# tyiannak/pyAudioAnalysis

Hardware: NVIDIA H100
Metric: audio frames/sec short-term feature_extraction @16kHz 50/25ms (higher is better)
Workload: dtype f32

## Files before the change

### pyaudioanalysis_b200/csrc/b200aa.cu

```cuda
#include <cuda_runtime.h>
#include <nvtx3/nvToolsExt.h>

#include <algorithm>
#include <atomic>
#include <cmath>
#include <cstdio>
#include <cstring>
#include <map>
#include <memory>
#include <mutex>
#include <string>
#include <vector>

#include "../../include/b200aa.h"
#include "common.cuh"
#include "generic_kernel.cuh"
#include "fast_kernel.cuh"
#include "pair_kernel.cuh"
#include "solo_kernel.cuh"
#include "tables.inl"

using namespace b200aa;

static thread_local std::string g_cuda_err;
// ... 236 lines not shown
                if (cntg[g] < 3 && (best < 0 || load[g] < load[best])) best = g;
            grp[best * 3 + cntg[best]++] = f;
            load[best] += m_count[f];
        }
        bl.mel_grp = put_i(grp);
    }
    while (blob.size() % 4) blob.push_back(0);
    bl.words = (int)blob.size();
    return (rc_mel != B200AA_OK) ? rc_mel : rc_chr;
}

extern "C" int b200aa_plan_create(b200aa_plan **out, int fs, int window, int step)
{
    if (!out || fs <= 0 || window < 2 || step < 1) return B200AA_ERR_INVALID;
    int rc = b200aa_device_ok();
    if (rc != B200AA_OK) return rc;
    std::unique_ptr<b200aa_plan> pl(new b200aa_plan);
    pl->fs = fs; pl->window = window; pl->step = step; pl->K = window / 2;
    CK(cudaGetDevice(&pl->device));
    CK(cudaDeviceGetAttribute(&pl->sm_count, cudaDevAttrMultiProcessorCount, pl->device));
    pl->tables_status = build_blob(fs, pl->K, pl->h_blob, pl->bl);
    CK(cudaMalloc(&pl->d_blob, sizeof(int) * pl->h_blob.size()));
    CK(cudaMemcpy(pl->d_blob, pl->h_blob.data(), sizeof(int) * pl->h_blob.size(), cudaMemcpyHostToDevice));
    Transform *t = nullptr;
    rc = get_transform(pl.get(), window, &t);
    if (rc != B200AA_OK) return rc;
    rc = fast_plan_init(fs, window, step, pl->h_blob, pl->bl, &pl->fast, &pl->fast_kind);
    if (rc != B200AA_OK) return rc;
    int sl_ = 0, sr_ = 0;
    if ((pair_r_for_window(window) || solo_shape_for_window(window, &sl_, &sr_)) && pl->tables_status == B200AA_OK) {
        std::vector<double> mel, chr, dct;
        b200aa_host::build_mel(fs, pl->K, mel);
        b200aa_host::build_chroma(fs, pl->K, chr);
        b200aa_host::build_dct(dct);
        std::vector<int> pblob;
        PairBlobLayout pbl{};
        build_pair_blob(mel, chr, dct, pl->K, pblob, pbl);
        rc = pair_plan_init(window, pblob, pbl, &pl->pair);
        if (rc != B200AA_OK) return cuda_fail(cudaGetLastError(), "pair_plan_init");
        rc = solo_plan_init(window, pblob, pbl, &pl->solo);
        if (rc != B200AA_OK) return cuda_fail(cudaGetLastError(), "solo_plan_init");
    }
    CK(cudaMalloc(&pl->d_counters, b200aa_plan::kSlots * b200aa_plan::kSlotBytes));
    *out = pl.release();
    return B200AA_OK;
}

extern "C" void b200aa_plan_destroy(b200aa_plan *plan) { delete plan; }
static int slot_acquire(b200aa_plan *pl, cudaStream_t st, unsigned *slot, unsigned int **ctr)
{
    std::lock_guard<std::mutex> g(pl->slot_mu);
    const unsigned s = pl->next_slot++ % b200aa_plan::kSlots;
    if (!pl->slot_event[s]) CK(cudaEventCreateWithFlags(&pl->slot_event[s], cudaEventDisableTiming));
    if (pl->slot_used[s]) CK(cudaStreamWaitEvent(st, pl->slot_event[s], 0));
    *slot = s;
    *ctr = reinterpret_cast<unsigned int *>(pl->d_counters + size_t(s) * b200aa_plan::kSlotBytes);
    return B200AA_OK;
}
static int slot_done(b200aa_plan *pl, cudaStream_t st, unsigned slot)
{
    std::lock_guard<std::mutex> g(pl->slot_mu);
    CK(cudaEventRecord(pl->slot_event[slot], st));
    pl->slot_used[slot] = true;
    return B200AA_OK;
}

static bool use_pair(const b200aa_plan *pl) { return pl->pair.R && !pl->force_generic && (pl->prefer < 0 || pl->prefer == 2); }
static bool use_solo(const b200aa_plan *pl) { return pl->solo.L && !pl->force_generic && (pl->prefer < 0 || pl->prefer == 3); }
static bool use_fast(const b200aa_plan *pl) { return pl->fast_kind && !pl->force_generic && (pl->prefer < 0 || pl->prefer == 1); }
extern "C" int b200aa_plan_kernel_kind(const b200aa_plan *plan)
{
    if (!plan) return 0;
    return use_pair(plan) ? 2 : (use_solo(plan) ? 3 : (use_fast(plan) ? 1 : 0));
}
extern "C" int b200aa_plan_prefer_kernel(b200aa_plan *plan, int kind)
{
    if (!plan || kind < -1 || kind > 3) return B200AA_ERR_INVALID;
    plan->prefer = kind;
    return B200AA_OK;
}
static float *g_pair_dump = nullptr;
extern "C" int b200aa_debug_set_dump(float *d_rows)
{
    g_pair_dump = d_rows;
    return B200AA_OK;
}
extern "C" int b200aa_plan_force_generic(b200aa_plan *plan, int on)
{
    if (!plan) return 0;
    int prev = plan->force_generic;
    plan->force_generic = on ? 1 : 0;
    return prev;
}

extern "C" int b200aa_plan_trim(b200aa_plan *plan)
{
    if (!plan) return B200AA_ERR_INVALID;
    std::lock_guard<std::mutex> g(plan->host_mu);
    for (int i = 0; i < 4; ++i) {
        if (plan->ws[i]) cudaFree(plan->ws[i]);
        plan->ws[i] = nullptr; plan->ws_cap[i] = 0;
    }
    for (int k = 0; k < b200aa_plan::kPipe; ++k)
        for (int j = 0; j < 3; ++j) {
            if (plan->pipe_ws[k][j]) cudaFree(plan->pipe_ws[k][j]);
            plan->pipe_ws[k][j] = nullptr; plan->pipe_cap[k][j] = 0;
        }
    return B200AA_OK;
}

static int plan_device_check(const b200aa_plan *pl)
{
    int dev = -1;
    CK(cudaGetDevice(&dev));
    return dev == pl->device ? B200AA_OK : B200AA_ERR_INVALID;
}

__device__ __forceinline__ int float_key(float f)
{
    int b = __float_as_int(f);
    return b >= 0 ? b : b ^ 0x7fffffff;
}
__device__ __forceinline__ float key_float(int k) { return __int_as_float(k >= 0 ? k : k ^ 0x7fffffff); }

__global__ void stats_init_kernel(b200aa_clip_norm *nm, int64_t n)
{
    int64_t i = blockIdx.x * int64_t(blockDim.x) + threadIdx.x;
    if (i >= n) return;
    unsigned long long *acc = reinterpret_cast<unsigned long long *>(&nm[i].rsv[1]);
    *acc = 0ull;
    reinterpret_cast<int *>(&nm[i].lo)[0] = 0x7fffffff;
    reinterpret_cast<int *>(&nm[i].hi)[0] = int(0x80000000u);
}

template <int DTYPE>
__global__ void __launch_bounds__(256) stats_accum_kernel(const void *sig, int64_t n_samples, int64_t clip_stride,
                                                           const int64_t *len, b200aa_clip_norm *nm, int chunks)
{
    const int64_t b = blockIdx.y;
    const int64_t L = len ? len[b] : n_samples;
    const int64_t per = (L + chunks - 1) / chunks;
    const int64_t s0 = blockIdx.x * per, s1 = min(L, s0 + per);
    long long isum = 0;
    double dsum = 0.0;
    int kmin = 0x7fffffff, kmax = int(0x80000000u);
    if (DTYPE == B200AA_DTYPE_I16) {
        const short *x = reinterpret_cast<const short *>(sig) + b * clip_stride;
        int mn = 32767, mx = -32768;
        int64_t i = s0 + threadIdx.x;
        const bool al = ((reinterpret_cast<uintptr_t>(x + s0) & 15) == 0);
        if (al) {
            const int4 *v = reinterpret_cast<const int4 *>(x + s0);
            const int64_t nv = (s1 - s0) / 8;
            int64_t j = threadIdx.x;
            for (; j + 3 * int64_t(blockDim.x) < nv; j += 4 * int64_t(blockDim.x)) {
                int4 q[4];
#pragma unroll
                for (int t = 0; t < 4; ++t) q[t] = __ldg(v + j + t * int64_t(blockDim.x));
                int acc = 0;
#pragma unroll
                for (int t = 0; t < 4; ++t) {
                    const int w4[4] = {q[t].x, q[t].y, q[t].z, q[t].w};
#pragma unroll
                    for (int u = 0; u < 4; ++u) {
                        const int a0 = (short)(w4[u] & 0xffff), a1 = w4[u] >> 16;
                        acc += a0 + a1;
                        mn = min(mn, min(a0, a1));
                        mx = max(mx, max(a0, a1));
// ... 699 lines not shown
```

### pyaudioanalysis_b200/csrc/pair_kernel.cuh

```cuda
#pragma once
#include "common.cuh"
#include "dft_codelets.cuh"
#include <algorithm>
#include <cstring>
#include <utility>
#include "fast_kernel.cuh"
#include "sched.cuh"

namespace b200aa {

#ifndef B200AA_PAIR_MAXWARPS
#define B200AA_PAIR_MAXWARPS 24
#endif
constexpr int kPairMaxWarps = B200AA_PAIR_MAXWARPS;
#ifndef B200AA_PAIR_MINBLOCKS
#define B200AA_PAIR_MINBLOCKS 1
#endif
constexpr int kPairMinBlocks = B200AA_PAIR_MINBLOCKS;
#ifndef B200AA_SOLO_MAXWARPS
#define B200AA_SOLO_MAXWARPS 24
#endif
#ifndef B200AA_SOLO_MINBLOCKS
#define B200AA_SOLO_MINBLOCKS 1
#endif
// ... 201 lines not shown
        below += run > thr ? 0.f : 1.f;
#endif
    }
    const float sp = sp2.x + sp2.y, fl = fl2.x + fl2.y;
    __syncwarp();
    float e = 0.f;
    constexpr int MAXP = 2 * (Lb / CB + 2);
#pragma unroll
    for (int q = 0; q < MAXP; ++q) e += (dlv.y + q < dlv.z) ? parts[dlv.y + q] : 0.f;
    float ent = 0.f;
    if (l < 10) {
        const float sj = fdiv(e, sxx + B200AA_EPS);
        ent = -sj * flog2(sj + B200AA_EPS);
    }
    float q4;
    {
        const bool up8 = l & 8, up4 = l & 4;
        float k0_ = up8 ? below : sp, k1_ = up8 ? ent : fl;
        const float g0_ = up8 ? sp : below, g1_ = up8 ? fl : ent;
        k0_ += __shfl_xor_sync(0xffffffffu, g0_, 8);
        k1_ += __shfl_xor_sync(0xffffffffu, g1_, 8);
        float kk = up4 ? k1_ : k0_;
        const float gg = up4 ? k0_ : k1_;
        kk += __shfl_xor_sync(0xffffffffu, gg, 4);
        kk += __shfl_xor_sync(0xffffffffu, kk, 2);
        kk += __shfl_xor_sync(0xffffffffu, kk, 1);
        q4 = kk;
    }
    if (l == 0) {
        fv[3] = cen;
        fv[4] = sx > 0.f ? fsqrt_pos(fdiv(q4, sx)) : 0.f;
        fv[34] = sx;
        fv[35] = sxx;
    }
    if (l == 4) fv[6] = q4;
    if (l == 8) fv[7] = q4 >= float(K) ? 0.f : q4 * invK;
    if (l == 12) fv[5] = q4;
    __syncwarp();
}

template <int P, int NV, int D, int NA>
__device__ __forceinline__ void mr_halve(float (&v)[NA], int lane)
{
    if constexpr (P > 1) {
        constexpr int H = P / 2;
        const bool up = lane & D;
#pragma unroll
        for (int i = 0; i < H; ++i) {
            if (i < NV) {
                if (i + H < NV) {
                    const float keep = up ? v[i + H] : v[i], send = up ? v[i] : v[i + H];
                    v[i] = keep + __shfl_xor_sync(0xffffffffu, send, D);
                } else {
                    v[i] += __shfl_xor_sync(0xffffffffu, v[i], D);
                }
            }
        }
        mr_halve<H, (NV < H ? NV : H), D / 2, NA>(v, lane);
    } else {
#pragma unroll
        for (int d = D; d >= 1; d >>= 1) v[0] += __shfl_xor_sync(0xffffffffu, v[0], d);
    }
}
template <int NV>
struct MultiReduce {
    static constexpr int P0 = NV > 16 ? 32 : (NV > 8 ? 16 : 8);
    static constexpr int SH = NV > 16 ? 0 : (NV > 8 ? 1 : 2);
    __device__ static __forceinline__ void run(float (&v)[NV], int lane) { mr_halve<P0, NV, 16, NV>(v, lane); }
};

template <int R, bool FULL>
struct TdShape {
    using S = PairShape<R>;
    static constexpr int NREST = (S::N % 10) ? 1 : 0;
    static constexpr int NE = FULL ? 10 + NREST : 5;
    static constexpr int EB = FULL ? 0 : 5;
    static constexpr int NFIRST = FULL ? 0 : S::N / 2;
    static constexpr int ROW0 = NFIRST / 32, LANE0 = NFIRST % 32;
    static constexpr int ZROW0 = (!FULL && LANE0 == 0) ? ROW0 - 1 : ROW0;
    static_assert(FULL || S::kShareable, "half-frame sharing needs whole blocks per half");
};

template <int R, bool FULL, bool TWO>
__device__ __forceinline__ void td_frame(const float (&u)[R], float cm, const b200aa_clip_norm &nm, int lane,
                                         float *e , int &flips, int &link)
{
    using S = PairShape<R>;
    using Td = TdShape<R, FULL>;
    constexpr int N = S::N, Lt = S::Lt;
    unsigned prevP = 0u, prevQ = 0u;
    int fl = 0, lk = 0;
#pragma unroll
    for (int r = Td::ZROW0; r < R; ++r) {
        const float d = u[r] - cm;
        const unsigned P = __ballot_sync(0xffffffffu, d > nm.lo);
        unsigned Q = 0u;
        if (TWO) Q = __ballot_sync(0xffffffffu, d < nm.hi);
        if (FULL && r == 0) { prevP = (P & 1u) << 31; prevQ = (Q & 1u) << 31; }
        if (r >= Td::ROW0) {
            const int n0 = 32 * r;
            const int nstart = FULL ? 1 : Td::NFIRST;
            const unsigned valid = n0 >= nstart ? 0xffffffffu : (n0 + 32 <= nstart ? 0u : (0xffffffffu << (nstart - n0)));
            const unsigned cP = (P ^ __funnelshift_l(prevP, P, 1)) & valid;
            fl += __popc(cP);
            if (!FULL && r == Td::ROW0) lk += int((cP >> Td::LANE0) & 1u);
            if (TWO) {
                const unsigned cQ = (Q ^ __funnelshift_l(prevQ, Q, 1)) & valid;
                fl += __popc(cQ);
                if (!FULL && r == Td::ROW0) lk += int((cQ >> Td::LANE0) & 1u);
            }
            const float y = fmaf(nm.a, d, nm.bp);
            const bool live = !(r == Td::ROW0 && Td::LANE0 > 0) || lane >= Td::LANE0;
            const int b0 = (n0 / Lt) < 10 ? (n0 / Lt) : 10;
            const int end = b0 < 10 ? (b0 + 1) * Lt : N;
            const int thr = end - n0;
            const int i0 = b0 - Td::EB, i1 = (b0 + 1 < 10 ? b0 + 1 : 10) - Td::EB;
            if (thr >= 32) {
                if (i0 >= 0 && i0 < Td::NE) { if (live) e[i0] = fmaf(y, y, e[i0]); }
            } else {
                const bool first = lane < thr;
                if (i0 >= 0 && i0 < Td::NE) { if (live && first) e[i0] = fmaf(y, y, e[i0]); }
                if (i1 >= 0 && i1 < Td::NE) { if (live && !first) e[i1] = fmaf(y, y, e[i1]); }
            }
        }
        prevP = P; prevQ = Q;
    }
    flips = TWO ? fl : 2 * fl;
    link = TWO ? lk : 2 * lk;
}

template <int R, bool FULL, bool TWO>
__device__ __forceinline__ void td_pair(const float2 (&u)[R], float cm, const b200aa_clip_norm &nm, int lane,
                                        float2 *e2 , int &flips_a, int &link_a, int &flips_b, int &link_b)
{
    using S = PairShape<R>;
    using Td = TdShape<R, FULL>;
    constexpr int N = S::N, Lt = S::Lt;
    unsigned pPa = 0u, pQa = 0u, pPb = 0u, pQb = 0u;
    int fa = 0, la = 0, fb = 0, lb = 0;
    const float2 ncm = make_float2(-cm, -cm), a2 = make_float2(nm.a, nm.a), bp2 = make_float2(nm.bp, nm.bp);
#pragma unroll
    for (int r = Td::ZROW0; r < R; ++r) {
        const float2 d = f2add(u[r], ncm);
        const unsigned Pa = __ballot_sync(0xffffffffu, d.x > nm.lo), Pb = __ballot_sync(0xffffffffu, d.y > nm.lo);
        unsigned Qa = 0u, Qb = 0u;
        if (TWO) { Qa = __ballot_sync(0xffffffffu, d.x < nm.hi); Qb = __ballot_sync(0xffffffffu, d.y < nm.hi); }
        if (FULL && r == 0) { pPa = (Pa & 1u) << 31; pQa = (Qa & 1u) << 31; pPb = (Pb & 1u) << 31; pQb = (Qb & 1u) << 31; }
        if (r >= Td::ROW0) {
            const int n0 = 32 * r;
            const int nstart = FULL ? 1 : Td::NFIRST;
            const unsigned valid = n0 >= nstart ? 0xffffffffu : (n0 + 32 <= nstart ? 0u : (0xffffffffu << (nstart - n0)));
            const unsigned cPa = (Pa ^ __funnelshift_l(pPa, Pa, 1)) & valid, cPb = (Pb ^ __funnelshift_l(pPb, Pb, 1)) & valid;
            fa += __popc(cPa); fb += __popc(cPb);
            if (!FULL && r == Td::ROW0) { la += int((cPa >> Td::LANE0) & 1u); lb += int((cPb >> Td::LANE0) & 1u); }
            if (TWO) {
                const unsigned cQa = (Qa ^ __funnelshift_l(pQa, Qa, 1)) & valid, cQb = (Qb ^ __funnelshift_l(pQb, Qb, 1)) & valid;
                fa += __popc(cQa); fb += __popc(cQb);
                if (!FULL && r == Td::ROW0) { la += int((cQa >> Td::LANE0) & 1u); lb += int((cQb >> Td::LANE0) & 1u); }
            }
            const float2 y = f2fma(a2, d, bp2);
            const bool live = !(r == Td::ROW0 && Td::LANE0 > 0) || lane >= Td::LANE0;
            const int b0 = (n0 / Lt) < 10 ? (n0 / Lt) : 10;
            const int end = b0 < 10 ? (b0 + 1) * Lt : N;
            const int thr = end - n0;
            const int i0 = b0 - Td::EB, i1 = (b0 + 1 < 10 ? b0 + 1 : 10) - Td::EB;
            if (thr >= 32) {
                if (i0 >= 0 && i0 < Td::NE) { if (live) e2[i0] = f2fma(y, y, e2[i0]); }
            } else {
                const bool first = lane < thr;
                if (i0 >= 0 && i0 < Td::NE) { if (live && first) e2[i0] = f2fma(y, y, e2[i0]); }
                if (i1 >= 0 && i1 < Td::NE) { if (live && !first) e2[i1] = f2fma(y, y, e2[i1]); }
            }
        }
        pPa = Pa; pQa = Qa; pPb = Pb; pQb = Qb;
    }
    flips_a = TWO ? fa : 2 * fa; link_a = TWO ? la : 2 * la;
    flips_b = TWO ? fb : 2 * fb; link_b = TWO ? lb : 2 * lb;
}

__device__ __forceinline__ void frame_scale(float E, float inv_a2n, float &s, float &inv_s)
{
    const float t = E * inv_a2n;
    const int ex = (__float_as_int(t) >> 23) & 0xff;
    int k = (127 - ex) >> 1;
    k = k < -30 ? -30 : (k > 40 ? 40 : k);
    s = __int_as_float((127 + k) << 23);
    inv_s = __int_as_float((127 - k) << 23);
}

struct FeatTables {
    const float *dct;
    const int *mrec;
    const float4 *mw;
    const int2 *chr;
    int LQ, CT;
};

template <int K>
__device__ __forceinline__ void rows_to_features(const float *Xa, const float *Xb, const float *Xprev, bool fresh, float carried,
                                                 const int *dlane, float *parts, float *msraw, float *mslog, float *mfold, float *chr,
                                                 float *fva, float *fvb, const FeatTables &ft, int lane)
{
    const int half = lane >> 4, l16 = lane & 15;
    const unsigned FULLM = 0xffffffffu;
    {
        const float *X = half ? Xb : Xa;
        const float *Xp = half ? Xa : Xprev;
        pair_spectral<K>(X, Xp, carried, fresh, dlane + l16 * 4, parts + half * 32, half ? fvb : fva, l16, half);
    }
    {
        const float *X = half ? Xb : Xa;
        float acc = 0.f;
#pragma unroll 4
        for (int q = 0; q < ft.LQ; ++q) {
            const int rec = ft.mrec[q * 16 + l16];
            const float4 w = ft.mw[q * 16 + l16];
            const float *xp = X + (rec & 0xffff);
            acc = fmaf(xp[0], w.x, acc);
            acc = fmaf(xp[1], w.y, acc);
            acc = fmaf(xp[2], w.z, acc);
            acc = fmaf(xp[3], w.w, acc);
            if (rec & (1 << 24)) { msraw[half * B200AA_N_MEL + ((rec >> 16) & 0xff)] = acc; acc = 0.f; }
        }
        float ch = 0.f;
        for (int t = 0; t < ft.CT; ++t) {
            const int2 e = ft.chr[t * 16 + l16];
            const float v = X[e.x];
            ch = fmaf(v * v, __int_as_float(e.y), ch);
        }
        if (l16 < 12) chr[half * 12 + l16] = ch;
    }
    __syncwarp();
#pragma unroll
    for (int t = lane; t < 2 * B200AA_N_MEL; t += 32) mslog[t] = 0.30102999566398120f * flog2(msraw[t] + B200AA_EPS);
    __syncwarp();
#pragma unroll
    for (int t = lane; t < 2 * B200AA_N_MEL; t += 32) {
        const int f = t >= B200AA_N_MEL ? 1 : 0, r = t - f * B200AA_N_MEL;
        const int kind = r >= 20 ? 1 : 0, n = r - 20 * kind;
        const float *m = mslog + f * B200AA_N_MEL;
        const float a = m[n], bq = m[39 - n], kap = m[0];
        mfold[t] = kind ? a - bq : (a - kap) + (bq - kap);
    }
    __syncwarp();
    {
        const int c = l16 < B200AA_N_MFCC ? l16 : 0;
        const float *src = mfold + half * B200AA_N_MEL + 20 * (c & 1);
        const float *row = ft.dct + c * 41;
        float acc = 0.f;
#pragma unroll
        for (int n = 0; n < 20; ++n) acc = fmaf(row[n], src[n], acc);
        if (c == 0) acc = fmaf(6.324555320336759f, mslog[half * B200AA_N_MEL], acc);
        if (l16 < B200AA_N_MFCC) (half ? fvb : fva)[8 + c] = acc;
    }
    chroma_finalize_h(chr + half * 12, half ? fvb : fva, l16, true);
    __syncwarp();
    (void)FULLM;
}

__device__ __forceinline__ void tile_store(const float *fv, int tile_n, int tile_t0, float *out_clip, int64_t t_stride, int n_out, int lane)
{
    const int c = lane & 7, f0 = lane >> 3;
    if (c < tile_n) {
        float *const out_b = out_clip + tile_t0 + c;
        const float *cur_row = fv + (1 + c) * kFvStride, *prv_row = fv + c * kFvStride;
        const bool first = tile_t0 + c == 0;
#pragma unroll
        for (int i = 0; i < 9; ++i) {
            const int f = f0 + 4 * i;
            if (f < B200AA_N_BASE) {
                const float v = cur_row[f];
                out_b[size_t(f) * t_stride] = v;
                if (n_out > B200AA_N_BASE) out_b[size_t(f + B200AA_N_BASE) * t_stride] = first ? 0.f : v - prv_row[f];
            }
        }
    }
}

__device__ __forceinline__ void tile_flush(float *fv, int &tile_n, int &tile_t0, float *out_clip, int64_t t_stride, int n_out, int lane)
{
    if (tile_n > 0) {
        tile_store(fv, tile_n, tile_t0, out_clip, t_stride, n_out, lane);
        __syncwarp();
        fv[lane] = fv[tile_n * kFvStride + lane];
        if (lane < 4) fv[32 + lane] = fv[tile_n * kFvStride + 32 + lane];
        tile_t0 += tile_n;
        tile_n = 0;
        __syncwarp();
    }
}

template <int R, bool SHARED>
__global__ void __launch_bounds__(32 * pair_warps<R>(), kPairMinBlocks) st_pair_kernel(const PairParams pp)
{
    using S = PairShape<R>;
    constexpr int N = S::N, K = S::K, Kp = S::Kp, C = S::C, JK = S::JK, LS = S::LS;
    static_assert(!SHARED || S::kShareable, "shared halves need N % 160 == 0");
    extern __shared__ __align__(16) unsigned char smem_raw[];
    PairCtaMem<R> &cm_ = *reinterpret_cast<PairCtaMem<R> *>(smem_raw);
    int *const blob_s = reinterpret_cast<int *>(smem_raw + sizeof(PairCtaMem<R>));
    const StParams &p = pp.st;
    const int tid = threadIdx.x, lane = tid & 31, warp = tid >> 5;
    constexpr int NTHR = 32 * pair_warps<R>();
    for (int i = tid; i < pp.pbl.words; i += NTHR) blob_s[i] = pp.pblob[i];
    for (int i = tid; i < R * 32; i += NTHR) cm_.tw[i] = pp.tw[i];
    if (tid < 16) *reinterpret_cast<int4 *>(cm_.dlane + tid * 4) = pair_lane_init<K>(tid);
    __syncthreads();
    const float *const t_dct = reinterpret_cast<const float *>(blob_s + pp.pbl.dct);
    const int *const t_mrec = blob_s + pp.pbl.mel_rec;
    const float4 *const t_mw = reinterpret_cast<const float4 *>(blob_s + pp.pbl.mel_w);
    const int2 *const t_chr = reinterpret_cast<const int2 *>(blob_s + pp.pbl.chr);
    const FeatTables ftab{t_dct, t_mrec, t_mw, t_chr, pp.pbl.lq, pp.pbl.ct};
    PairWarpMem<R> &wm = cm_.w[warp];
    float *const rowa = reinterpret_cast<float *>(wm.tz);
    float *const t_re = reinterpret_cast<float *>(wm.tz), *const t_im = t_re + R * LS;
    float *const msraw = rowa + S::MS0, *const mslog = msraw + 2 * B200AA_N_MEL, *const mfold = mslog + 2 * B200AA_N_MEL;
    const int step = p.step;
    const int half = lane >> 4, l16 = lane & 15;
    const unsigned FULLM = 0xffffffffu;

    const unsigned wglob = blockIdx.x * unsigned(pair_warps<R>()) + unsigned(warp);
    if (lane == 0) sched_begin(pp.sched, wglob);
    __syncwarp();
    const int per_clip = int(pp.sched.per_clip);
    unsigned run_b = 0xffffffffu, run_q = 0xffffffffu;
    int tile_n = 0, tile_t0 = 0;
    int zprev = 0;
#define B200AA_PAIR_FLUSH(clip_index) tile_flush(wm.fv, tile_n, tile_t0, p.out + size_t(clip_index) * p.n_out * p.t_stride, p.t_stride, p.n_out, lane)

    unsigned inc = pp.sched.chunk;
    for (;;) {
        unsigned g0 = 0, g1 = 0;
        const int got = sched_next(pp.sched, blockIdx.x * unsigned(pair_warps<R>()) + unsigned(warp), lane, inc, g0, g1);
        if (got == 0) break;
        if (got == 2) continue;
        while (g0 < g1) {
        const unsigned cb = g0 / unsigned(per_clip);
        const int q0 = int(g0 - cb * unsigned(per_clip));
        int qe = q0 + int(g1 - g0);
        qe = qe < per_clip ? qe : per_clip;
        const int64_t b = int64_t(cb);
        const bool cont = cb == run_b && unsigned(q0) == run_q;
        if (!cont) B200AA_PAIR_FLUSH(run_b);
        const int64_t len = p.len ? p.len[b] : p.n_samples;
        const int T = int(len < N ? 0 : (len - N) / step + 1);
        const int NP = (T + 1) >> 1;
        const b200aa_clip_norm nm = p.norm[b];
        const bool is16 = p.dtype == B200AA_DTYPE_I16;
        const char *const clip = reinterpret_cast<const char *>(p.sig) + size_t(b) * p.clip_stride * (is16 ? 2 : 4);
        const float M0 = is16 ? 8421376.f : 0.f;
        const float cmv = M0 + nm.m;
        const bool two_sided = !(nm.hi > nm.lo);
        const float inv_a2n = 1.f / (nm.a * nm.a * float(N));
        const float fscale = nm.a * (0.5f / float(K));
        bool fresh = !cont;
        if (!cont) {
            tile_t0 = 2 * q0;
            zprev = 0;
        }
        g0 += unsigned(qe - q0);
        run_b = cb;
        run_q = 0xffffffffu;
        if (q0 >= NP) continue;
        const int q1 = qe < NP ? qe : NP;
        auto load_pair = [&](int qq, unsigned int (&wa)[R], unsigned int (&wb)[R]) {
            const int ta_ = 2 * qq, tb_ = (ta_ + 1 < T) ? ta_ + 1 : ta_;
            if (is16) {
                const unsigned short *pa = reinterpret_cast<const unsigned short *>(clip) + size_t(ta_) * step + lane;
                const unsigned short *pb = reinterpret_cast<const unsigned short *>(clip) + size_t(tb_) * step + lane;
#pragma unroll
                for (int r = 0; r < R; ++r) { wa[r] = __ldg(pa + 32 * r); wb[r] = __ldg(pb + 32 * r); }
            } else {
                const unsigned int *pa = reinterpret_cast<const unsigned int *>(clip) + size_t(ta_) * step + lane;
                const unsigned int *pb = reinterpret_cast<const unsigned int *>(clip) + size_t(tb_) * step + lane;
#pragma unroll
                for (int r = 0; r < R; ++r) { wa[r] = __ldg(pa + 32 * r); wb[r] = __ldg(pb + 32 * r); }
            }
        };
        for (int q = q0 - ((fresh && q0 > 0) ? 1 : 0); q < q1; ++q) {
            const bool store = q >= q0;
            const int ta = 2 * q;
            const bool bvalid = ta + 1 < T;
            float2 uab[R];
            {
                unsigned int wa[R], wb[R];
                load_pair(q, wa, wb);
                if (is16) {
#pragma unroll
                    for (int r = 0; r < R; ++r)
                        uab[r] = make_float2(__int_as_float(0x4B000000 | (int(wa[r]) ^ 0x8000)), __int_as_float(0x4B000000 | (int(wb[r]) ^ 0x8000)));
                } else {
#pragma unroll
                    for (int r = 0; r < R; ++r) uab[r] = make_float2(__int_as_float(wa[r]), __int_as_float(wb[r]));
                }
            }
            const float u0a = __shfl_sync(FULLM, uab[0].x, 0), u0b = __shfl_sync(FULLM, uab[0].y, 0);
            const int ra = store ? 1 + tile_n : 8, rb = store ? 2 + tile_n : 0;
            float *const fva = wm.fv + ra * kFvStride, *const fvb = wm.fv + rb * kFvStride;

            const bool a_full = !SHARED || fresh;
            int fl_a, fl_b;
            {
                constexpr int NEF = TdShape<R, true>::NE, NREST = TdShape<R, true>::NREST;
                if constexpr (SHARED) { if (!a_full) {
                    float2 e2[5];
#pragma unroll
                    for (int i = 0; i < 5; ++i) e2[i] = make_float2(0.f, 0.f);
                    int fa_, la_, fb_, lb_;
                    if (two_sided) td_pair<R, false, true>(uab, cmv, nm, lane, e2, fa_, la_, fb_, lb_);
                    else td_pair<R, false, false>(uab, cmv, nm, lane, e2, fa_, la_, fb_, lb_);
                    float ev[10];
#pragma unroll
                    for (int i = 0; i < 5; ++i) { ev[i] = e2[i].x; ev[5 + i] = e2[i].y; }
                    if (lane < 5) wm.blk[lane] = wm.blk[10 + lane];
                    MultiReduce<10>::run(ev, lane);
                    __syncwarp();
                    if ((lane & 1) == 0 && (lane >> 1) < 10) wm.blk[5 + (lane >> 1)] = ev[0];
                    fl_a = zprev + fa_;
                    fl_b = (fa_ - la_) + fb_;
                    zprev = fb_ - lb_;
                } else {
                    float ua[R], ub[R];
#pragma unroll
                    for (int r = 0; r < R; ++r) { ua[r] = uab[r].x; ub[r] = uab[r].y; }
                    float ev[NEF + 5];
#pragma unroll
                    for (int i = 0; i < NEF + 5; ++i) ev[i] = 0.f;
                    int fa_, la_, fb_, lb_;
                    if (two_sided) { td_frame<R, true, true>(ua, cmv, nm, lane, ev, fa_, la_); td_frame<R, false, true>(ub, cmv, nm, lane, ev + NEF, fb_, lb_); }
                    else { td_frame<R, true, false>(ua, cmv, nm, lane, ev, fa_, la_); td_frame<R, false, false>(ub, cmv, nm, lane, ev + NEF, fb_, lb_); }
                    int fh_, lh_;
                    { float dump[5] = {0.f, 0.f, 0.f, 0.f, 0.f};
                      if (two_sided) td_frame<R, false, true>(ua, cmv, nm, lane, dump, fh_, lh_); else td_frame<R, false, false>(ua, cmv, nm, lane, dump, fh_, lh_); }
                    MultiReduce<NEF + 5>::run(ev, lane);
                    __syncwarp();
                    {
                        constexpr int SH = MultiReduce<NEF + 5>::SH;
                        const int j = lane >> SH;
                        if ((lane & ((1 << SH) - 1)) == 0 && j < NEF + 5) wm.blk[j] = ev[0];
                    }
                    fl_a = fa_;
                    fl_b = (fh_ - lh_) + fb_;
                    zprev = fb_ - lb_;
                } } else {
                    float2 e2[NEF];
#pragma unroll
                    for (int i = 0; i < NEF; ++i) e2[i] = make_float2(0.f, 0.f);
                    int la_, lb_;
                    if (two_sided) td_pair<R, true, true>(uab, cmv, nm, lane, e2, fl_a, la_, fl_b, lb_);
                    else td_pair<R, true, false>(uab, cmv, nm, lane, e2, fl_a, la_, fl_b, lb_);
                    float ev[2 * NEF];
#pragma unroll
                    for (int i = 0; i < NEF; ++i) { ev[i] = e2[i].x; ev[NEF + i] = e2[i].y; }
                    MultiReduce<2 * NEF>::run(ev, lane);
                    __syncwarp();
                    {
                        constexpr int SH = MultiReduce<2 * NEF>::SH;
                        const int j = lane >> SH;
                        if ((lane & ((1 << SH) - 1)) == 0 && j < 2 * NEF) {
                            const int f = j >= NEF ? 1 : 0, i = j - f * NEF;
                            wm.blk[i < 10 ? 10 * f + i : 20 + f] = ev[0];
                        }
                    }
                    (void)NREST;
                }
            }
            __syncwarp();
            float Ea, Eb;
            {
                constexpr int OB = SHARED ? 5 : 10;
                const bool own = l16 < 10;
                const float e = own ? wm.blk[half * OB + l16] : 0.f;
                float tot = half_sum(e);
                if (!SHARED && TdShape<R, true>::NREST) tot += wm.blk[20 + half];
                const float sj = fdiv(e, tot + B200AA_EPS);
                const float H = half_sum(own ? -sj * flog2(sj + B200AA_EPS) : 0.f);
                if (l16 == 0) {
                    float *fv = half ? fvb : fva;
                    fv[0] = float(half ? fl_b : fl_a) * 0.5f / float(N - 1);
                    fv[1] = tot / float(N);
                    fv[2] = H;
                }
                Ea = __shfl_sync(FULLM, tot, 0);
                Eb = __shfl_sync(FULLM, tot, 16);
            }

            float sa, isa, sb, isb;
            frame_scale(Ea, inv_a2n, sa, isa);
            frame_scale(Eb, inv_a2n, sb, isb);
            bool a_flat, b_flat;
            {
                float2 z[R];
                const float2 s2 = make_float2(sa, sb), o2 = make_float2(-u0a * sa, -u0b * sb);
                float2 zz = make_float2(0.f, 0.f);
#pragma unroll
                for (int r = 0; r < R; ++r) {
                    z[r] = f2fma(uab[r], s2, o2);
                    zz = f2fma(z[r], z[r], zz);
                }
                a_flat = !__any_sync(FULLM, zz.x > 0.f);
                b_flat = !__any_sync(FULLM, zz.y > 0.f);
                fft_r<R>(z);
                t_re[lane] = z[0].x; t_im[lane] = z[0].y;
#pragma unroll
                for (int k1 = 1; k1 < R; ++k1) {
                    const float2 w = cmul(z[k1], cm_.tw[k1 * 32 + lane]);
                    t_re[k1 * LS + lane] = w.x; t_im[k1 * LS + lane] = w.y;
                }
            }
            __syncwarp();
            {
                float2 v[32];
                {
                    float2 re[16], im[16];
                    const int row = lane < R ? lane : 0;
                    const float2 *pr = reinterpret_cast<const float2 *>(t_re + row * LS), *pi = reinterpret_cast<const float2 *>(t_im + row * LS);
#pragma unroll
                    for (int m = 0; m < 16; ++m) { re[m] = pr[m]; im[m] = pi[m]; }
                    fft32_soa(re, im, v);
                }
                __syncwarp();
                if (lane < R) {
#pragma unroll
                    for (int k2 = 0; k2 < 32; ++k2) wm.tz[lane + R * k2] = v[k2];
                    if (lane == 0) wm.tz[N] = v[0];
                }
            }
            __syncwarp();
            float xa[C], xb[C];
            {
                const float fa = a_flat ? 0.f : fscale * isa, fb = b_flat ? 0.f : fscale * isb;
#pragma unroll
                for (int j = 0; j < C; ++j) {
                    const int k = lane + 32 * j;
                    xa[j] = 0.f; xb[j] = 0.f;
                    if (j < JK && k < K) {
                        const float2 zk = wm.tz[k], pk = wm.tz[N - k];
                        const float2 sm_ = f2add(zk, pk), df_ = f2sub(zk, pk);
                        xa[j] = fsqrt_fast(fmaf(sm_.x, sm_.x, df_.y * df_.y)) * fa;
                        xb[j] = fsqrt_fast(fmaf(df_.x, df_.x, sm_.y * sm_.y)) * fb;
                    }
                }
                if (lane == 0) {
                    const float2 z0 = wm.tz[0];
                    xa[0] = fabsf(fmaf(nm.a * isa, z0.x, float(N) * fmaf(nm.a, u0a - cmv, nm.bp))) / float(K);
                    xb[0] = fabsf(fmaf(nm.a * isb, z0.y, float(N) * fmaf(nm.a, u0b - cmv, nm.bp))) / float(K);
                }
            }
            __syncwarp();
            float *const rowbn = rowa + S::RB0;
#pragma unroll
            for (int j = 0; j < C; ++j) { rowa[lane + 32 * j] = xa[j]; rowbn[lane + 32 * j] = xb[j]; }
            if (pp.dbg) {
#pragma unroll
                for (int j = 0; j < JK; ++j) {
                    const int k = lane + 32 * j;
                    if (k < K) {
                        pp.dbg[(size_t(b) * p.t_stride + ta) * K + k] = xa[j];
                        if (bvalid) pp.dbg[(size_t(b) * p.t_stride + ta + 1) * K + k] = xb[j];
                    }
                }
            }
            __syncwarp();
            rows_to_features<K>(rowa, rowbn, fresh ? rowa : wm.rowp, fresh, wm.fv[(ra - 1) * kFvStride + 34], cm_.dlane,
                                rowa + S::PT0, msraw, mslog, mfold, rowa + S::CH0, fva, fvb, ftab, lane);
#pragma unroll
            for (int j = 0; j < (Kp / 4 + 31) / 32; ++j) {
                const int i4 = lane + 32 * j;
                if (i4 < Kp / 4) reinterpret_cast<float4 *>(wm.rowp)[i4] = reinterpret_cast<const float4 *>(rowbn)[i4];
            }

            if (store) {
                tile_n += bvalid ? 2 : 1;
                if (tile_n == 8) B200AA_PAIR_FLUSH(cb);
            }
            fresh = false;
            __syncwarp();
        }
        if (q1 < NP) run_q = unsigned(q1);
        else B200AA_PAIR_FLUSH(cb);
        }
    }
    B200AA_PAIR_FLUSH(run_b);
#undef B200AA_PAIR_FLUSH
}

inline int pair_r_for_window(int window)
{
    switch (window) {
    case 320: return 10;
    case 480: return 15;
    case 512: return 16;
    case 640: return 20;
    case 800: return 25;
    case 960: return 30;
    case 1024: return 32;
    default: return 0;
    }
}

struct PairTables {
    float2 *d_tw = nullptr;
    int *d_pblob = nullptr;
    PairBlobLayout pbl{};
    int R = 0;
    void release()
    {
        if (d_tw) cudaFree(d_tw);
        if (d_pblob) cudaFree(d_pblob);
        d_tw = nullptr; d_pblob = nullptr;
    }
};

inline void build_pair_blob(const std::vector<double> &mel, const std::vector<double> &chr, const std::vector<double> &dct, int K,
                            std::vector<int> &blob, PairBlobLayout &bl)
{
    struct Quad { int start, fid, last; float w[4]; };
    std::vector<std::vector<Quad>> per_filter(B200AA_N_MEL);
    for (int i = 0; i < B200AA_N_MEL; ++i) {
        int lo = -1, hi = -1;
        if (!mel.empty())
            for (int k = 0; k < K; ++k)
                if (mel[size_t(i) * K + k] != 0.0) { if (lo < 0) lo = k; hi = k; }
        if (lo < 0) { lo = 0; hi = -1; }
        const int nq = hi >= lo ? (hi - lo + 4) / 4 : 1;
        for (int q = 0; q < nq; ++q) {
            Quad qd{};
            const int s = lo + 4 * q;
            int s2 = s;
            if (s2 + 4 > K) s2 = K - 4 > 0 ? K - 4 : 0;
            qd.start = s2; qd.fid = i; qd.last = q == nq - 1;
            for (int j = 0; j < 4; ++j) {
                const int k = s2 + j;
                qd.w[j] = (k >= s && k < s + 4 && k <= hi && k < K) ? float(mel[size_t(i) * K + k]) : 0.f;
            }
            per_filter[i].push_back(qd);
        }
    }
    std::vector<int> order(B200AA_N_MEL);
    for (int i = 0; i < B200AA_N_MEL; ++i) order[i] = i;
    std::stable_sort(order.begin(), order.end(), [&](int a, int b) { return per_filter[a].size() > per_filter[b].size(); });
    std::vector<std::vector<Quad>> lanes(16);
    for (int i : order) {
        int best = 0;
        for (int l = 1; l < 16; ++l) if (lanes[l].size() < lanes[best].size()) best = l;
        lanes[best].insert(lanes[best].end(), per_filter[i].begin(), per_filter[i].end());
    }
    size_t lq = 1;
    for (auto &l : lanes) lq = l.size() > lq ? l.size() : lq;
    std::vector<std::vector<std::pair<int, float>>> taps(12);
    size_t ct = 1;
    if (!chr.empty())
        for (int c = 0; c < 12; ++c) {
            for (int k = 0; k < K; ++k)
                if (chr[size_t(c) * K + k] != 0.0) taps[c].push_back({k, float(chr[size_t(c) * K + k])});
            ct = taps[c].size() > ct ? taps[c].size() : ct;
        }
    auto fbits = [](float f) { int w; std::memcpy(&w, &f, 4); return w; };
    blob.clear();
    bl.dct = 0;
    blob.resize(13 * 41 + 3, 0);
    for (int r = 0; r < 13; ++r)
        for (int n = 0; n < 40; ++n) blob[r * 41 + n] = fbits(float(dct[size_t(r) * 40 + n]));
    while (blob.size() % 4) blob.push_back(0);
    bl.mel_rec = (int)blob.size();
    for (size_t q = 0; q < lq; ++q)
        for (int l = 0; l < 16; ++l) {
            int rec = 0;
            if (q < lanes[l].size()) rec = lanes[l][q].start | (lanes[l][q].fid << 16) | (lanes[l][q].last << 24);
            blob.push_back(rec);
        }
    bl.mel_w = (int)blob.size();
    for (size_t q = 0; q < lq; ++q)
        for (int l = 0; l < 16; ++l)
            for (int j = 0; j < 4; ++j) blob.push_back(q < lanes[l].size() ? fbits(lanes[l][q].w[j]) : 0);
    bl.chr = (int)blob.size();
    for (size_t t = 0; t < ct; ++t)
        for (int l = 0; l < 16; ++l) {
            const bool have = l < 12 && t < taps[l].size();
            blob.push_back(have ? taps[l][t].first : 0);
            blob.push_back(have ? fbits(taps[l][t].second) : 0);
        }
    while (blob.size() % 4) blob.push_back(0);
    bl.lq = (int)lq; bl.ct = (int)ct;
    bl.words = (int)blob.size();
}

inline int pair_plan_init(int window, const std::vector<int> &h_pblob, const PairBlobLayout &pbl, PairTables *pt)
{
    const int R = pair_r_for_window(window);
    pt->R = 0;
    if (!R) return B200AA_OK;
    if (getenv("B200AA_NO_PAIR")) return B200AA_OK;
    const int N = 32 * R;
    const double pi = 3.14159265358979323846264338327950288;
    std::vector<float2> tw(size_t(R) * 32);
    for (int k1 = 0; k1 < R; ++k1)
        for (int n2 = 0; n2 < 32; ++n2) {
            const double a = -2.0 * pi * double((k1 * n2) % N) / double(N);
            tw[size_t(k1) * 32 + n2] = make_float2(float(std::cos(a)), float(std::sin(a)));
        }
    if (cudaMalloc(&pt->d_tw, tw.size() * sizeof(float2)) != cudaSuccess) return B200AA_ERR_CUDA;
    if (cudaMemcpy(pt->d_tw, tw.data(), tw.size() * sizeof(float2), cudaMemcpyHostToDevice) != cudaSuccess) return B200AA_ERR_CUDA;
    if (cudaMalloc(&pt->d_pblob, h_pblob.size() * sizeof(int)) != cudaSuccess) return B200AA_ERR_CUDA;
    if (cudaMemcpy(pt->d_pblob, h_pblob.data(), h_pblob.size() * sizeof(int), cudaMemcpyHostToDevice) != cudaSuccess) return B200AA_ERR_CUDA;
    pt->pbl = pbl;
    pt->R = R;
    return B200AA_OK;
}

#ifndef B200AA_LAYOUT_ONLY
template <int R, bool SHARED>
inline int pair_launch_t(const PairTables &pt, const StParams &p, int sm_count, int64_t T, unsigned long long *ranges, size_t ranges_cap,
                         float *dbg, cudaStream_t st)
{
    const size_t smem = pair_smem_bytes<R>(pt.pbl.words);
    if (smem > size_t(kPairCtaCap)) return B200AA_ERR_UNSUPPORTED;
    auto kern = st_pair_kernel<R, SHARED>;
    if (cudaFuncSetAttribute(kern, cudaFuncAttributeMaxDynamicSharedMemorySize, kPairCtaCap) != cudaSuccess) return B200AA_ERR_CUDA;
    int occ = 1;
    if (cudaOccupancyMaxActiveBlocksPerMultiprocessor(&occ, kern, 32 * pair_warps<R>(), smem) != cudaSuccess) return B200AA_ERR_CUDA;
    occ = occ < 1 ? 1 : occ;
    PairParams pp;
    pp.st = p;
    pp.tw = pt.d_tw;
    pp.pblob = pt.d_pblob;
    pp.pbl = pt.pbl;
    pp.dbg = dbg;
    const int64_t NP = (T + 1) / 2;
    constexpr int kPairWarps = pair_warps<R>();
    const int64_t total = NP * p.n_clips;
    if (total <= 0) return B200AA_OK;
    if (total >= (int64_t(1) << 31)) return B200AA_ERR_UNSUPPORTED;
    int64_t grid = int64_t(sm_count) * occ;
    if (grid * kPairWarps > total) grid = (total + kPairWarps - 1) / kPairWarps;
    const int64_t n_warps = grid * kPairWarps;
    if (size_t(n_warps) * sizeof(unsigned long long) > ranges_cap) return B200AA_ERR_UNSUPPORTED;
    long chunk = 8, min_steal = 2;
    if (const char *ov = getenv("B200AA_PAIR_STEAL")) {
        long a = 0, b2 = 0;
        if (sscanf(ov, "%ld,%ld", &a, &b2) == 2 && a > 0 && a <= 65536 && b2 > 1 && b2 <= 65536) { chunk = a; min_steal = b2; }
    }
    pp.sched.ranges = ranges;
    pp.sched.n_warps = unsigned(n_warps);
    pp.sched.total = unsigned(total);
    pp.sched.per_clip = unsigned(NP);
    pp.sched.chunk = unsigned(chunk);
    pp.sched.min_steal = unsigned(min_steal);
    pp.st.n_items = total;
    if (getenv("B200AA_DEBUG"))
        fprintf(stderr, "[b200aa] pair kernel R=%d shared=%d: smem %zu B, %d CTAs/SM x %d warps, grid %lld, %lld pairs (%lld per clip), chunk %ld, min steal %ld\n",
                R, int(SHARED), smem, occ, kPairWarps, (long long)grid, (long long)total, (long long)NP, chunk, min_steal);
    if (cudaMemsetAsync(ranges, 0, size_t(n_warps) * sizeof(unsigned long long), st) != cudaSuccess) return B200AA_ERR_CUDA;
    kern<<<(unsigned)grid, 32 * kPairWarps, smem, st>>>(pp);
    return cudaPeekAtLastError() == cudaSuccess ? B200AA_OK : B200AA_ERR_CUDA;
}

template <int R>
inline int pair_launch_r(const PairTables &pt, const StParams &p, int sm_count, int64_t T, unsigned long long *ranges, size_t ranges_cap,
                         float *dbg, cudaStream_t st)
{
    constexpr int N = 32 * R;
    if (PairShape<R>::kShareable && p.step == N / 2) return pair_launch_t<R, PairShape<R>::kShareable>(pt, p, sm_count, T, ranges, ranges_cap, dbg, st);
    return pair_launch_t<R, false>(pt, p, sm_count, T, ranges, ranges_cap, dbg, st);
}

inline int pair_launch_features(const PairTables &pt, const StParams &p, int sm_count, int64_t T, unsigned long long *ranges, size_t ranges_cap,
                                float *dbg, cudaStream_t st)
{
    switch (pt.R) {
    case 10: return pair_launch_r<10>(pt, p, sm_count, T, ranges, ranges_cap, dbg, st);
    case 15: return pair_launch_r<15>(pt, p, sm_count, T, ranges, ranges_cap, dbg, st);
    case 16: return pair_launch_r<16>(pt, p, sm_count, T, ranges, ranges_cap, dbg, st);
    case 32: return pair_launch_r<32>(pt, p, sm_count, T, ranges, ranges_cap, dbg, st);
    case 20: return pair_launch_r<20>(pt, p, sm_count, T, ranges, ranges_cap, dbg, st);
    case 25: return pair_launch_r<25>(pt, p, sm_count, T, ranges, ranges_cap, dbg, st);
    case 30: return pair_launch_r<30>(pt, p, sm_count, T, ranges, ranges_cap, dbg, st);
    default: return B200AA_ERR_UNSUPPORTED;
    }
}
#endif

}
```

Measured before the change: 350.0 million.

## Compute first-half zero crossings cheaply, compile out debug dump, retune steal chunk

Replaces the separate full-frame td_frame path for an uncached first half with a lightweight td_first_half routine that runs on top of the shared pair computation. This drops redundant per-frame ballot and energy work and removes a code path. The debug row dump is now compiled only under a macro, which takes a runtime branch out of the hot loop. Optional clock64-based phase instrumentation is added but is off by default. The work-steal chunk for large windows (R>=25) is raised, trading finer load balance for fewer atomics.

```diff
diff --git a/pyaudioanalysis_b200/csrc/b200aa.cu b/pyaudioanalysis_b200/csrc/b200aa.cu
--- a/pyaudioanalysis_b200/csrc/b200aa.cu
+++ b/pyaudioanalysis_b200/csrc/b200aa.cu
@@ -342,8 +342,26 @@
 static float *g_pair_dump = nullptr;
 extern "C" int b200aa_debug_set_dump(float *d_rows)
 {
+#ifdef B200AA_PAIR_DUMP
     g_pair_dump = d_rows;
     return B200AA_OK;
+#else
+    return d_rows ? B200AA_ERR_UNSUPPORTED : B200AA_OK;
+#endif
+}
+extern "C" int b200aa_debug_pair_phase_clocks(unsigned long long *out, int reset)
+{
+#ifdef B200AA_PAIR_PHASE_CLOCKS
+    if (out && cudaMemcpyFromSymbol(out, b200aa::g_pair_phase_clocks, sizeof(b200aa::g_pair_phase_clocks)) != cudaSuccess) return B200AA_ERR_CUDA;
+    if (reset) {
+        static const unsigned long long zero[b200aa::kPairPhases + 1] = {};
+        if (cudaMemcpyToSymbol(b200aa::g_pair_phase_clocks, zero, sizeof(zero)) != cudaSuccess) return B200AA_ERR_CUDA;
+    }
+    return B200AA_OK;
+#else
+    (void)out; (void)reset;
+    return B200AA_ERR_UNSUPPORTED;
+#endif
 }
 extern "C" int b200aa_plan_force_generic(b200aa_plan *plan, int on)
 {
diff --git a/pyaudioanalysis_b200/csrc/pair_kernel.cuh b/pyaudioanalysis_b200/csrc/pair_kernel.cuh
--- a/pyaudioanalysis_b200/csrc/pair_kernel.cuh
+++ b/pyaudioanalysis_b200/csrc/pair_kernel.cuh
@@ -307,54 +307,6 @@
 };
 
 template <int R, bool FULL, bool TWO>
-__device__ __forceinline__ void td_frame(const float (&u)[R], float cm, const b200aa_clip_norm &nm, int lane,
-                                         float *e , int &flips, int &link)
-{
-    using S = PairShape<R>;
-    using Td = TdShape<R, FULL>;
-    constexpr int N = S::N, Lt = S::Lt;
-    unsigned prevP = 0u, prevQ = 0u;
-    int fl = 0, lk = 0;
-#pragma unroll
-    for (int r = Td::ZROW0; r < R; ++r) {
-        const float d = u[r] - cm;
-        const unsigned P = __ballot_sync(0xffffffffu, d > nm.lo);
-        unsigned Q = 0u;
-        if (TWO) Q = __ballot_sync(0xffffffffu, d < nm.hi);
-        if (FULL && r == 0) { prevP = (P & 1u) << 31; prevQ = (Q & 1u) << 31; }
-        if (r >= Td::ROW0) {
-            const int n0 = 32 * r;
-            const int nstart = FULL ? 1 : Td::NFIRST;
-            const unsigned valid = n0 >= nstart ? 0xffffffffu : (n0 + 32 <= nstart ? 0u : (0xffffffffu << (nstart - n0)));
-            const unsigned cP = (P ^ __funnelshift_l(prevP, P, 1)) & valid;
-            fl += __popc(cP);
-            if (!FULL && r == Td::ROW0) lk += int((cP >> Td::LANE0) & 1u);
-            if (TWO) {
-                const unsigned cQ = (Q ^ __funnelshift_l(prevQ, Q, 1)) & valid;
-                fl += __popc(cQ);
-                if (!FULL && r == Td::ROW0) lk += int((cQ >> Td::LANE0) & 1u);
-            }
-            const float y = fmaf(nm.a, d, nm.bp);
-            const bool live = !(r == Td::ROW0 && Td::LANE0 > 0) || lane >= Td::LANE0;
-            const int b0 = (n0 / Lt) < 10 ? (n0 / Lt) : 10;
-            const int end = b0 < 10 ? (b0 + 1) * Lt : N;
-            const int thr = end - n0;
-            const int i0 = b0 - Td::EB, i1 = (b0 + 1 < 10 ? b0 + 1 : 10) - Td::EB;
-            if (thr >= 32) {
-                if (i0 >= 0 && i0 < Td::NE) { if (live) e[i0] = fmaf(y, y, e[i0]); }
-            } else {
-                const bool first = lane < thr;
-                if (i0 >= 0 && i0 < Td::NE) { if (live && first) e[i0] = fmaf(y, y, e[i0]); }
-                if (i1 >= 0 && i1 < Td::NE) { if (live && !first) e[i1] = fmaf(y, y, e[i1]); }
-            }
-        }
-        prevP = P; prevQ = Q;
-    }
-    flips = TWO ? fl : 2 * fl;
-    link = TWO ? lk : 2 * lk;
-}
-
-template <int R, bool FULL, bool TWO>
 __device__ __forceinline__ void td_pair(const float2 (&u)[R], float cm, const b200aa_clip_norm &nm, int lane,
                                         float2 *e2 , int &flips_a, int &link_a, int &flips_b, int &link_b)
 {
@@ -403,6 +355,41 @@
     flips_b = TWO ? fb : 2 * fb; link_b = TWO ? lb : 2 * lb;
 }
 
+template <int R, bool TWO>
+__device__ __forceinline__ void td_first_half(const float2 (&u)[R], float cm, const b200aa_clip_norm &nm, int lane,
+                                              float *e , int &flips)
+{
+    using S = PairShape<R>;
+    constexpr int NH = S::N / 2, Lt = S::Lt, RE = (NH + 31) / 32;
+    static_assert(S::kShareable, "half a frame = 5 whole blocks");
+    unsigned prevP = 0u, prevQ = 0u;
+    int fl = 0;
+#pragma unroll
+    for (int r = 0; r < RE; ++r) {
+        const float d = __fadd_rn(u[r].x, -cm);
+        const unsigned P = __ballot_sync(0xffffffffu, d > nm.lo);
+        unsigned Q = 0u;
+        if (TWO) Q = __ballot_sync(0xffffffffu, d < nm.hi);
+        if (r == 0) { prevP = (P & 1u) << 31; prevQ = (Q & 1u) << 31; }
+        const int n0 = 32 * r;
+        const unsigned valid = n0 + 32 <= NH ? 0xffffffffu : (0xffffffffu >> (n0 + 32 - NH));
+        fl += __popc((P ^ __funnelshift_l(prevP, P, 1)) & valid);
+        if (TWO) fl += __popc((Q ^ __funnelshift_l(prevQ, Q, 1)) & valid);
+        const float y = __fmaf_rn(nm.a, d, nm.bp);
+        const bool live = n0 + 32 <= NH || lane < NH - n0;
+        const int b0 = n0 / Lt, thr = (b0 + 1) * Lt - n0;
+        if (thr >= 32) {
+            if (live) e[b0] = __fmaf_rn(y, y, e[b0]);
+        } else {
+            const bool first = lane < thr;
+            if (live && first) e[b0] = __fmaf_rn(y, y, e[b0]);
+            if (b0 + 1 < 5) { if (live && !first) e[b0 + 1] = __fmaf_rn(y, y, e[b0 + 1]); }
+        }
+        prevP = P; prevQ = Q;
+    }
+    flips = TWO ? fl : 2 * fl;
+}
+
 __device__ __forceinline__ void frame_scale(float E, float inv_a2n, float &s, float &inv_s)
 {
     const float t = E * inv_a2n;
@@ -421,10 +408,52 @@
     int LQ, CT;
 };
 
-template <int K>
+enum PairPhase { kPhLoad, kPhTime, kPhPass1, kPhPass2, kPhSep, kPhSpectral, kPhMel, kPhChroma, kPhStore, kPhSched, kPairPhases };
+
+struct NoPhaseClock {
+    __device__ __forceinline__ void mark(int) {}
+};
+#ifdef B200AA_PAIR_PHASE_CLOCKS
+__device__ unsigned long long g_pair_phase_clocks[kPairPhases + 1];
+struct PairPhaseClock {
+    unsigned acc[kPairPhases];
+    long long t;
+    unsigned steps;
+    __device__ __forceinline__ void start()
+    {
+#pragma unroll
+        for (int i = 0; i < kPairPhases; ++i) acc[i] = 0u;
+        steps = 0u;
+        t = clock64();
+    }
+    __device__ __forceinline__ void mark(int ph)
+    {
+        const long long n = clock64();
+        acc[ph] += unsigned(n - t);
+        t = n;
+    }
+    __device__ __forceinline__ void step() { ++steps; }
+    __device__ __forceinline__ void finish(int lane)
+    {
+        if (lane == 0) {
+#pragma unroll
+            for (int i = 0; i < kPairPhases; ++i) atomicAdd(&g_pair_phase_clocks[i], (unsigned long long)acc[i]);
+            atomicAdd(&g_pair_phase_clocks[kPairPhases], (unsigned long long)steps);
+        }
+    }
+};
+#else
+struct PairPhaseClock : NoPhaseClock {
+    __device__ __forceinline__ void start() {}
+    __device__ __forceinline__ void step() {}
+    __device__ __forceinline__ void finish(int) {}
+};
+#endif
+
+template <int K, class Clock = NoPhaseClock>
 __device__ __forceinline__ void rows_to_features(const float *Xa, const float *Xb, const float *Xprev, bool fresh, float carried,
                                                  const int *dlane, float *parts, float *msraw, float *mslog, float *mfold, float *chr,
-                                                 float *fva, float *fvb, const FeatTables &ft, int lane)
+                                                 float *fva, float *fvb, const FeatTables &ft, int lane, Clock &&clk = Clock())
 {
     const int half = lane >> 4, l16 = lane & 15;
     const unsigned FULLM = 0xffffffffu;
@@ -433,6 +462,7 @@
         const float *Xp = half ? Xa : Xprev;
         pair_spectral<K>(X, Xp, carried, fresh, dlane + l16 * 4, parts + half * 32, half ? fvb : fva, l16, half);
     }
+    clk.mark(kPhSpectral);
     {
         const float *X = half ? Xb : Xa;
         float acc = 0.f;
@@ -447,6 +477,7 @@
             acc = fmaf(xp[3], w.w, acc);
             if (rec & (1 << 24)) { msraw[half * B200AA_N_MEL + ((rec >> 16) & 0xff)] = acc; acc = 0.f; }
         }
+        clk.mark(kPhMel);
         float ch = 0.f;
         for (int t = 0; t < ft.CT; ++t) {
             const int2 e = ft.chr[t * 16 + l16];
@@ -456,6 +487,7 @@
         if (l16 < 12) chr[half * 12 + l16] = ch;
     }
     __syncwarp();
+    clk.mark(kPhChroma);
 #pragma unroll
     for (int t = lane; t < 2 * B200AA_N_MEL; t += 32) mslog[t] = 0.30102999566398120f * flog2(msraw[t] + B200AA_EPS);
     __syncwarp();
@@ -478,8 +510,10 @@
         if (c == 0) acc = fmaf(6.324555320336759f, mslog[half * B200AA_N_MEL], acc);
         if (l16 < B200AA_N_MFCC) (half ? fvb : fva)[8 + c] = acc;
     }
+    clk.mark(kPhMel);
     chroma_finalize_h(chr + half * 12, half ? fvb : fva, l16, true);
     __syncwarp();
+    clk.mark(kPhChroma);
     (void)FULLM;
 }
 
@@ -554,6 +588,8 @@
 #define B200AA_PAIR_FLUSH(clip_index) tile_flush(wm.fv, tile_n, tile_t0, p.out + size_t(clip_index) * p.n_out * p.t_stride, p.t_stride, p.n_out, lane)
 
     unsigned inc = pp.sched.chunk;
+    PairPhaseClock clk;
+    clk.start();
     for (;;) {
         unsigned g0 = 0, g1 = 0;
         const int got = sched_next(pp.sched, blockIdx.x * unsigned(pair_warps<R>()) + unsigned(warp), lane, inc, g0, g1);
@@ -566,7 +602,9 @@
         qe = qe < per_clip ? qe : per_clip;
         const int64_t b = int64_t(cb);
         const bool cont = cb == run_b && unsigned(q0) == run_q;
+        clk.mark(kPhSched);
         if (!cont) B200AA_PAIR_FLUSH(run_b);
+        clk.mark(kPhStore);
         const int64_t len = p.len ? p.len[b] : p.n_samples;
         const int T = int(len < N ? 0 : (len - N) / step + 1);
         const int NP = (T + 1) >> 1;
@@ -579,10 +617,7 @@
         const float inv_a2n = 1.f / (nm.a * nm.a * float(N));
         const float fscale = nm.a * (0.5f / float(K));
         bool fresh = !cont;
-        if (!cont) {
-            tile_t0 = 2 * q0;
-            zprev = 0;
-        }
+        if (!cont) tile_t0 = 2 * q0;
         g0 += unsigned(qe - q0);
         run_b = cb;
         run_q = 0xffffffffu;
@@ -603,6 +638,8 @@
             }
         };
         for (int q = q0 - ((fresh && q0 > 0) ? 1 : 0); q < q1; ++q) {
+            clk.mark(kPhSched);
+            clk.step();
             const bool store = q >= q0;
             const int ta = 2 * q;
             const bool bvalid = ta + 1 < T;
@@ -620,6 +657,7 @@
                 }
             }
             const float u0a = __shfl_sync(FULLM, uab[0].x, 0), u0b = __shfl_sync(FULLM, uab[0].y, 0);
+            clk.mark(kPhLoad);
             const int ra = store ? 1 + tile_n : 8, rb = store ? 2 + tile_n : 0;
             float *const fva = wm.fv + ra * kFvStride, *const fvb = wm.fv + rb * kFvStride;
 
@@ -627,17 +665,25 @@
             int fl_a, fl_b;
             {
                 constexpr int NEF = TdShape<R, true>::NE, NREST = TdShape<R, true>::NREST;
-                if constexpr (SHARED) { if (!a_full) {
+                if constexpr (SHARED) {
                     float2 e2[5];
 #pragma unroll
                     for (int i = 0; i < 5; ++i) e2[i] = make_float2(0.f, 0.f);
                     int fa_, la_, fb_, lb_;
                     if (two_sided) td_pair<R, false, true>(uab, cmv, nm, lane, e2, fa_, la_, fb_, lb_);
                     else td_pair<R, false, false>(uab, cmv, nm, lane, e2, fa_, la_, fb_, lb_);
+                    if (!a_full) {
+                        if (lane < 5) wm.blk[lane] = wm.blk[10 + lane];
+                    } else {
+                        float eh[5] = {0.f, 0.f, 0.f, 0.f, 0.f};
+                        if (two_sided) td_first_half<R, true>(uab, cmv, nm, lane, eh, zprev);
+                        else td_first_half<R, false>(uab, cmv, nm, lane, eh, zprev);
+                        MultiReduce<5>::run(eh, lane);
+                        if ((lane & 3) == 0 && (lane >> 2) < 5) wm.blk[lane >> 2] = eh[0];
+                    }
                     float ev[10];
 #pragma unroll
                     for (int i = 0; i < 5; ++i) { ev[i] = e2[i].x; ev[5 + i] = e2[i].y; }
-                    if (lane < 5) wm.blk[lane] = wm.blk[10 + lane];
                     MultiReduce<10>::run(ev, lane);
                     __syncwarp();
                     if ((lane & 1) == 0 && (lane >> 1) < 10) wm.blk[5 + (lane >> 1)] = ev[0];
@@ -645,29 +691,6 @@
                     fl_b = (fa_ - la_) + fb_;
                     zprev = fb_ - lb_;
                 } else {
-                    float ua[R], ub[R];
-#pragma unroll
-                    for (int r = 0; r < R; ++r) { ua[r] = uab[r].x; ub[r] = uab[r].y; }
-                    float ev[NEF + 5];
-#pragma unroll
-                    for (int i = 0; i < NEF + 5; ++i) ev[i] = 0.f;
-                    int fa_, la_, fb_, lb_;
-                    if (two_sided) { td_frame<R, true, true>(ua, cmv, nm, lane, ev, fa_, la_); td_frame<R, false, true>(ub, cmv, nm, lane, ev + NEF, fb_, lb_); }
-                    else { td_frame<R, true, false>(ua, cmv, nm, lane, ev, fa_, la_); td_frame<R, false, false>(ub, cmv, nm, lane, ev + NEF, fb_, lb_); }
-                    int fh_, lh_;
-                    { float dump[5] = {0.f, 0.f, 0.f, 0.f, 0.f};
-                      if (two_sided) td_frame<R, false, true>(ua, cmv, nm, lane, dump, fh_, lh_); else td_frame<R, false, false>(ua, cmv, nm, lane, dump, fh_, lh_); }
-                    MultiReduce<NEF + 5>::run(ev, lane);
-                    __syncwarp();
-                    {
-                        constexpr int SH = MultiReduce<NEF + 5>::SH;
-                        const int j = lane >> SH;
-                        if ((lane & ((1 << SH) - 1)) == 0 && j < NEF + 5) wm.blk[j] = ev[0];
-                    }
-                    fl_a = fa_;
-                    fl_b = (fh_ - lh_) + fb_;
-                    zprev = fb_ - lb_;
-                } } else {
                     float2 e2[NEF];
 #pragma unroll
                     for (int i = 0; i < NEF; ++i) e2[i] = make_float2(0.f, 0.f);
@@ -709,6 +732,7 @@
                 Ea = __shfl_sync(FULLM, tot, 0);
                 Eb = __shfl_sync(FULLM, tot, 16);
             }
+            clk.mark(kPhTime);
 
             float sa, isa, sb, isb;
             frame_scale(Ea, inv_a2n, sa, isa);
@@ -734,6 +758,7 @@
                 }
             }
             __syncwarp();
+            clk.mark(kPhPass1);
             {
                 float2 v[32];
                 {
@@ -752,6 +777,7 @@
                 }
             }
             __syncwarp();
+            clk.mark(kPhPass2);
             float xa[C], xb[C];
             {
                 const float fa = a_flat ? 0.f : fscale * isa, fb = b_flat ? 0.f : fscale * isb;
@@ -776,6 +802,7 @@
             float *const rowbn = rowa + S::RB0;
 #pragma unroll
             for (int j = 0; j < C; ++j) { rowa[lane + 32 * j] = xa[j]; rowbn[lane + 32 * j] = xb[j]; }
+#ifdef B200AA_PAIR_DUMP
             if (pp.dbg) {
 #pragma unroll
                 for (int j = 0; j < JK; ++j) {
@@ -786,9 +813,11 @@
                     }
                 }
             }
+#endif
             __syncwarp();
+            clk.mark(kPhSep);
             rows_to_features<K>(rowa, rowbn, fresh ? rowa : wm.rowp, fresh, wm.fv[(ra - 1) * kFvStride + 34], cm_.dlane,
-                                rowa + S::PT0, msraw, mslog, mfold, rowa + S::CH0, fva, fvb, ftab, lane);
+                                rowa + S::PT0, msraw, mslog, mfold, rowa + S::CH0, fva, fvb, ftab, lane, clk);
 #pragma unroll
             for (int j = 0; j < (Kp / 4 + 31) / 32; ++j) {
                 const int i4 = lane + 32 * j;
@@ -801,12 +830,15 @@
             }
             fresh = false;
             __syncwarp();
+            clk.mark(kPhStore);
         }
         if (q1 < NP) run_q = unsigned(q1);
-        else B200AA_PAIR_FLUSH(cb);
-        }
-    }
+        }
+    }
+    clk.mark(kPhSched);
     B200AA_PAIR_FLUSH(run_b);
+    clk.mark(kPhStore);
+    clk.finish(lane);
 #undef B200AA_PAIR_FLUSH
 }
 
@@ -961,7 +993,7 @@
     if (grid * kPairWarps > total) grid = (total + kPairWarps - 1) / kPairWarps;
     const int64_t n_warps = grid * kPairWarps;
     if (size_t(n_warps) * sizeof(unsigned long long) > ranges_cap) return B200AA_ERR_UNSUPPORTED;
-    long chunk = 8, min_steal = 2;
+    long chunk = R >= 25 ? 64 : 8, min_steal = R >= 25 ? 4 : 2;
     if (const char *ov = getenv("B200AA_PAIR_STEAL")) {
         long a = 0, b2 = 0;
         if (sscanf(ov, "%ld,%ld", &a, &b2) == 2 && a > 0 && a <= 65536 && b2 > 1 && b2 <= 65536) { chunk = a; min_steal = b2; }
```

Measured after the change: 357.0 million, median of 6. 1.02x the previous value.
